# qianyizh/ElasticReconstruction

Hardware: AMD Instinct MI355X
Metric: depth frames/sec into 512^3 TSDF (640x480) (higher is better)
Workload: dtype f32; 1 GPU; configs[1]; frames_per_gpu=91800, volume_units_touched=122, warp=True, inputs=hbm_resident, parallelism=single GPU

## Files before the change

### elasticreconstruction_amd/_ffi.py

```python
import ctypes as C
import os

_HERE = os.path.dirname(os.path.abspath(__file__))
LIB_PATH = os.environ.get("ER_HIP_LIB") or os.path.join(_HERE, "liber_hip.so")

SYMBOLS = [
    "er_last_error", "er_device_count", "er_abi_version", "er_request_hw_queues", "er_host_alloc", "er_host_free", "er_host_copy_h2d", "er_device_alloc", "er_device_free", "er_device_copy_d2h",
    "er_tsdf_create", "er_tsdf_destroy", "er_tsdf_set_stream", "er_tsdf_synchronize",
    "er_tsdf_wait_event", "er_tsdf_reset", "er_tsdf_status", "er_tsdf_set_unit_shard", "er_unit_owner",
    "er_tsdf_scale_depth", "er_tsdf_reproject", "er_tsdf_integrate", "er_tsdf_integrate_frames", "er_tsdf_prepass_trace", "er_tsdf_set_zbuf_epoch",
    "er_tsdf_unit_count", "er_tsdf_unit_keys", "er_tsdf_read_unit", "er_tsdf_sum_weight",
    "er_tsdf_extract_world", "er_tsdf_extract_surface", "er_tsdf_extract_oriented", "er_tsdf_extract_mesh", "er_mc_table", "er_tsdf_extract_mesh_indexed", "er_mesh_components", "er_tsdf_extract_mesh_cleaned", "er_mesh_simplify", "er_tsdf_extract_mesh_simplified", "er_tsdf_import_world", "er_raycast_params_default", "er_tsdf_raycast", "er_tsdf_raycast_batch", "er_tsdf_export_weighted", "er_tsdf_import_weighted",
    "er_tsdf_export_raw", "er_tsdf_import_raw",
    "er_tsdf_color_enable", "er_tsdf_read_unit_color", "er_tsdf_write_unit_color", "er_tsdf_color_frames", "er_tsdf_reproject_color", "er_tsdf_sample_colors",
    "er_tsdf_band_sizes", "er_tsdf_export_band", "er_tsdf_merge_band", "er_tsdf_import_band", "er_tsdf_drop_units",
    "er_tsdf_set_profiling", "er_tsdf_get_profile", "er_tsdf_set_timeline", "er_tsdf_get_timeline",
    "er_comm_unique_id", "er_comm_create", "er_comm_create_local", "er_comm_create_loopback", "er_comm_destroy", "er_comm_rank", "er_comm_world",
    "er_tsdf_allreduce", "er_comm_merge_stats", "er_comm_merge_stats_owner", "er_frame_block",
    "er_cloud_create", "er_cloud_create_batch", "er_cloud_create_from_tsdf", "er_cloud_destroy", "er_cloud_size",
    "er_icp_count_inliers", "er_icp_align", "er_icp_align_trace", "er_find_correspondence",
    "er_icp_count_inliers_batch", "er_icp_align_batch", "er_find_correspondence_batch", "er_icp_release_workspaces", "er_registration_batch", "er_ransac_fitness_batch", "er_ransac_inliers",
    "er_features_create", "er_features_destroy", "er_features_size", "er_feature_knn", "er_ransac_hypotheses", "er_ransac_params_default", "er_ransac_align", "er_ransac_align_batch",
    "er_odom_params_default", "er_odom_create", "er_odom_destroy", "er_odom_align_pairs", "er_odom_track", "er_frame_to_model_align", "er_frames_to_models_align", "er_odom_linearize", "er_odom_read_maps", "er_odom_tables",
    "er_cloud_read", "er_cloud_voxel_grid", "er_cloud_estimate_normals", "er_fpfh_estimate", "er_features_dim", "er_features_read",
    "er_frag_params_default", "er_frag_create", "er_frag_destroy", "er_frag_lane_bytes", "er_frag_build", "er_frag_count", "er_frag_read",
# ... 72 lines not shown
    L.er_tsdf_create.argtypes = [C.c_int, C.c_int, fp, C.c_int, C.c_int, C.POINTER(vp)]
    L.er_tsdf_destroy.argtypes = [vp]
    L.er_tsdf_set_stream.argtypes = [vp, vp]
    L.er_tsdf_synchronize.argtypes = [vp]
    L.er_tsdf_wait_event.argtypes = [vp, vp]
    L.er_tsdf_reset.argtypes = [vp]
    L.er_tsdf_status.argtypes = [vp, ip, C.POINTER(C.c_long)]
    L.er_tsdf_set_unit_shard.argtypes = [vp, C.c_int, C.c_int]
    L.er_unit_owner.argtypes = [C.c_int, C.c_int]
    L.er_tsdf_scale_depth.argtypes = [vp, vp, vp]
    L.er_tsdf_reproject.argtypes = [vp, vp, vp, C.c_int, C.c_float, vp, vp]
    L.er_tsdf_integrate.argtypes = [vp, vp, vp]
    L.er_tsdf_integrate_frames.argtypes = [vp, C.c_int, vp, C.c_int, vp, C.POINTER(ErWarp)]
    if hasattr(L, "er_tsdf_prepass_trace"):
        L.er_tsdf_prepass_trace.argtypes = [vp, C.c_int, vp, C.c_int, vp, C.POINTER(ErWarp), vp, ip, vp, vp, vp, vp, vp, C.c_int, ip]
    if hasattr(L, "er_tsdf_set_zbuf_epoch"):
        L.er_tsdf_set_zbuf_epoch.argtypes = [vp, C.c_int, C.c_uint]
    L.er_tsdf_unit_count.argtypes = [vp, ip]
    L.er_tsdf_unit_keys.argtypes = [vp, vp]
    L.er_tsdf_read_unit.argtypes = [vp, C.c_int, vp, vp]
    L.er_tsdf_sum_weight.argtypes = [vp, dp]
    L.er_tsdf_extract_world.argtypes = [vp, vp, C.c_long, C.POINTER(C.c_long)]
    L.er_tsdf_extract_surface.argtypes = [vp, vp, C.c_long, C.POINTER(C.c_long)]
    if hasattr(L, "er_tsdf_extract_oriented"):
        L.er_tsdf_extract_oriented.argtypes = [vp, vp, vp, C.c_long, C.POINTER(C.c_long)]
    L.er_tsdf_extract_mesh.argtypes = [vp, vp, C.c_long, C.POINTER(C.c_long)]
    L.er_mc_table.argtypes = [vp]
    if hasattr(L, "er_tsdf_extract_mesh_indexed"):
        L.er_tsdf_extract_mesh_indexed.argtypes = [vp, vp, vp, C.c_long, vp, C.c_long, C.POINTER(C.c_long), C.POINTER(C.c_long)]
        L.er_tsdf_import_world.argtypes = [vp, vp, C.c_long, ip]
# ... 188 lines not shown
```

### elasticreconstruction_amd/csrc/er_tsdf.h

```cpp
#pragma once

#include "er_common.h"
#include "er_compact.h"
#include "er_mem.h"
#include "er_tsdf_math.h"

#include "../../include/er_hip.h"

#include <algorithm>
#include <cstdlib>
#include <functional>
#include <utility>
#include <vector>

namespace er_tsdf_k {
using namespace er;

constexpr int kBlock = 256;
constexpr int kEmptyKey = -1;
constexpr uint32_t kZEmpty = 0xFFFFFFFFu;
constexpr uint32_t kZEpochMax = 0xFFFFu;

enum { C_NUNITS = 0, C_NBATCH = 1 , C_POOL_OVERFLOW = 2, C_TABLE_FULL = 3, C_OUT_OF_RANGE = 4,
       C_NBATCH1 = 6, C_NBATCH2 = 7, C_ZERO_WRITE = 8 ,
// ... 39 lines not shown
    const uint16_t* __restrict__ depth, uint32_t* __restrict__ zbuf, int n_frames, int cols, int rows,
    Camera cam, CameraInv cami, const float* __restrict__ lambda, const double* __restrict__ T12, float* __restrict__ scaled,
    int* __restrict__ ht_key, int* __restrict__ ht_slot, unsigned long long* __restrict__ ht_mask, int cap_mask,
    int hash_shift, int* __restrict__ batch, int* __restrict__ nbatch,
    int* __restrict__ counters, float* __restrict__ tile_max, float* __restrict__ tile_lo, float* __restrict__ tile_lo_fine, int2 shard,
    uint32_t* __restrict__ lastzero, uint32_t* __restrict__ zfix, const int* __restrict__ zero_flag, uint32_t ztag);
extern template __global__ void k_prepare<true>(const uint16_t* __restrict__, uint32_t* __restrict__, int, int, int, Camera, CameraInv, const float* __restrict__, const double* __restrict__, float* __restrict__, int* __restrict__, int* __restrict__, unsigned long long* __restrict__, int, int, int* __restrict__, int* __restrict__, int* __restrict__, float* __restrict__, float* __restrict__, float* __restrict__, int2, uint32_t* __restrict__, uint32_t* __restrict__, const int* __restrict__, uint32_t);
extern template __global__ void k_prepare<false>(const uint16_t* __restrict__, uint32_t* __restrict__, int, int, int, Camera, CameraInv, const float* __restrict__, const double* __restrict__, float* __restrict__, int* __restrict__, int* __restrict__, unsigned long long* __restrict__, int, int, int* __restrict__, int* __restrict__, int* __restrict__, float* __restrict__, float* __restrict__, float* __restrict__, int2, uint32_t* __restrict__, uint32_t* __restrict__, const int* __restrict__, uint32_t);

constexpr int kRows = 4;
constexpr int kItemsPerUnit = 256;

struct Plan {
  int n_units;
  int next;
};

struct PlanRec {
  int key;
  int slot;
  unsigned long long mask;
};

constexpr int kIntMinBlocks = 5;

template <bool kSure>
__global__ __launch_bounds__(kBlock, kIntMinBlocks) void k_integrate(
    float2* __restrict__ pool, const PlanRec* __restrict__ plan_rec, Plan* __restrict__ plan,
    const FrameXform* __restrict__ frames, const float* __restrict__ scaled, const float* __restrict__ tile_max,
    const float* __restrict__ tile_lo, const float* __restrict__ tile_lo_fine, int tiles_x, int tiles_y, Camera cam, int cols, int rows);
extern template __global__ void k_integrate<true>(float2* __restrict__, const PlanRec* __restrict__, Plan* __restrict__, const FrameXform* __restrict__, const float* __restrict__, const float* __restrict__, const float* __restrict__, const float* __restrict__, int, int, Camera, int, int);
extern template __global__ void k_integrate<false>(float2* __restrict__, const PlanRec* __restrict__, Plan* __restrict__, const FrameXform* __restrict__, const float* __restrict__, const float* __restrict__, const float* __restrict__, const float* __restrict__, int, int, Camera, int, int);
}

struct er_tsdf_mem {
  er::DevScope fixed;
  er::Buffer<unsigned long long> color;
  er::Buffer<int> key_scratch, slot_scratch;
  er::Buffer<float> ctr_dev[2];
  er::Buffer<char> band_scratch;
  er::Buffer<char> color_scratch;
};

struct er_tsdf_s : er_tsdf_mem {
  int device = 0, cols = 0, rows = 0, pixels = 0, max_units = 0;
  er::Camera cam{};
  er::CameraInv cami{};
// ... 21 lines not shown
  er::PinnedBuffer<char> pinned[er_tsdf_k::kDepth];
  int ht_cap = 0, ht_shift = 0;
  float *lambda = nullptr, *ctr = nullptr;
  er::PinnedBuffer<float> ctr_pinned[2];
  hipEvent_t ctr_ev[2] = {nullptr, nullptr};
  hipEvent_t ctr_rd[2][er_tsdf_k::kAux] = {};
  bool ctr_rd_set[2] = {false, false};
  int ctr_parity = 0, ctr_cur = 0;
  uint16_t* depth_stage[er_tsdf_k::kDepth] = {};
  uint32_t *zbuf[er_tsdf_k::kAux] = {}, *lastzero[er_tsdf_k::kAux] = {}, *zfix[er_tsdf_k::kAux] = {};
  uint32_t zepoch[er_tsdf_k::kAux + 1] = {};
  double *T12 = nullptr, *seg12 = nullptr, *madj12 = nullptr, *dsum = nullptr;
  int* grid_index = nullptr;
  er_tsdf_k::PlanRec* plan_rec[er_tsdf_k::kDepth] = {};
  er_tsdf_k::Plan* plan[er_tsdf_k::kDepth] = {};
  int prof_stride = 0;
  long prof_tick = 0;
  std::vector<std::pair<hipEvent_t, hipEvent_t>> events;
  double ms_total = 0.0;
  long launches = 0, frames_done = 0;
  struct TimelineRow {
    long batch;
    int slot, stream, frames;
    double host_ms[3];
    hipEvent_t ev[7];
  };
  bool tl_on = false;
  hipEvent_t tl_base = nullptr;
  double tl_host0 = 0.0;
  std::vector<TimelineRow> tl_rows;
// ... 23 lines not shown
```

### elasticreconstruction_amd/csrc/er_tsdf.hip

```cpp
#include "er_tsdf_dev.h"

#include <chrono>
#include <climits>

namespace {

using namespace er_tsdf_k;

constexpr int kNbatchSlot[3] = {C_NBATCH, C_NBATCH1, C_NBATCH2};
constexpr int kZeroFlagSlot[2] = {C_ZERO_WRITE, C_ZERO_WRITE1};

__global__ void k_lambda(float* __restrict__ lambda, int cols, int rows, Camera cam) {
  int p = blockIdx.x * blockDim.x + threadIdx.x;
  if (p >= cols * rows) return;
  lambda[p] = scale_lambda(p % cols, p / cols, cam);
}

__global__ void k_scale_depth(const uint16_t* __restrict__ depth, const float* __restrict__ lambda,
                              float* __restrict__ scaled, int pixels, float itrunc) {
  int p = blockIdx.x * blockDim.x + threadIdx.x;
  if (p >= pixels) return;
  scaled[p] = scale_depth_px(depth[p], lambda[p], itrunc);
}

// ... 49 lines not shown
                                              int* __restrict__ zero_flag, unsigned long long* __restrict__ stats) {
  __shared__ int hist[65];
  __shared__ int start[66];
  const int n = *nbatch;
  for (int t = threadIdx.x; t < 65; t += blockDim.x) hist[t] = 0;
  __syncthreads();
  for (int t = threadIdx.x; t < n; t += blockDim.x) atomicAdd(&hist[__popcll(ht_mask[batch[t]])], 1);
  __syncthreads();
  if (threadIdx.x == 0) {
    int acc = 0;
    for (int c = 64; c >= 0; c--) {
      start[c] = acc;
      acc += hist[c];
    }
    plan->n_units = n;
    plan->next = 0;
    if (zero_flag) zero_flag[0] = zero_flag[1] = 0;
  }
  __syncthreads();
  if (threadIdx.x == 0) *nbatch = 0;
  unsigned long long visits = 0;
  for (int t = threadIdx.x; t < n; t += blockDim.x) {
    const int e = batch[t];
    const unsigned long long mask = ht_mask[e];
    ht_mask[e] = 0ull;
    visits += (unsigned long long)__popcll(mask);
    const int key = ht_key[e];
    PlanRec r;
    r.key = key;
    r.slot = unit_slot_acquire(e, key, ht_slot, unit_key, max_units, counters);
    r.mask = mask;
    plan_rec[atomicAdd(&start[__popcll(mask)], 1)] = r;
  }
  if (visits) atomicAdd(&stats[0], visits);
}

__global__ void k_sum_weight(const float2* __restrict__ pool, long n_vox, double* __restrict__ out) {
  double s = 0.0;
  for (long t = (long)blockIdx.x * blockDim.x + threadIdx.x; t < n_vox; t += (long)gridDim.x * blockDim.x)
    s += (double)pool[t].y;
  for (int off = 32; off > 0; off >>= 1) s += __shfl_down(s, off);
  __shared__ double part[kBlock / 64];
  if ((threadIdx.x & 63) == 0) part[threadIdx.x >> 6] = s;
  __syncthreads();
  if (threadIdx.x == 0) {
    double b = 0.0;
    for (int w = 0; w < kBlock / 64; w++) b += part[w];
    atomicAdd(out, b);
  }
// ... 218 lines not shown
      st->fx[f].mi[q] = (float)Tinv[q];
      st->t12[f * 12 + q] = Tf[q];
    }
    st->fx[f].tx = (float)Tf[3];
    st->fx[f].ty = (float)Tf[7];
    st->fx[f].tz = (float)Tf[11];
    st->fx[f].pad = 0.f;
    for (int q = 0; q < 16; q++) st->fxT[q][f] = reinterpret_cast<const float*>(&st->fx[f])[q];
  }
  static_assert(offsetof(Staging, fxT) == sizeof(er::FrameXform) * ER_MAX_BATCH && sizeof(er::FrameXform) == 64, "fxT lies directly behind fx");
  hipStream_t X = h->aux_stream[a], S = h->own_stream;
  int* nbatch = h->counters + kNbatchSlot[p];

  constexpr int kIntBlocksPerCu = 3;
  const int wide_grid = h->n_cu * kIntBlocksPerCu;
  uint32_t* zsrc = nullptr;
  char* dst = static_cast<char*>(h->dstage[p]);
  const double* dev_t12 = reinterpret_cast<const double*>(dst + offsetof(Staging, t12));
  const double* dev_seg = reinterpret_cast<const double*>(dst + offsetof(Staging, seg));
  const double* dev_madj = reinterpret_cast<const double*>(dst + offsetof(Staging, madj));
  const int* dev_gi = reinterpret_cast<const int*>(dst + offsetof(Staging, gi));
  if (warp) {
    for (int f = 0; f < n; f++) {
      for (int q = 0; q < 12; q++) {
        st->seg[f * 16 + q] = warp->seg[(size_t)(frame0 + f) * 16 + q];
        st->madj[f * 12 + q] = warp->madj[(size_t)(frame0 + f) * 16 + q];
      }
      er::cube_coord_deltas(&st->seg[f * 16], h->cam, h->cols, h->rows, &st->seg[f * 16 + 12]);
      st->seg[f * 16 + 15] = 0.0;
      const int g = warp->grid_index[frame0 + f];
// ... 18 lines not shown
    zsrc = h->zbuf[a];
  }
  if (tl && tl_record(h, &tl->ev[2], X)) return 1;

  const bool wide = h->cols % 4 == 0 && (zsrc || reinterpret_cast<uintptr_t>(depth_dev) % 8 == 0);
  hipLaunchKernelGGL(wide ? k_prepare<true> : k_prepare<false>, dim3((h->cols + kTile - 1) / kTile, (h->rows + kTile - 1) / kTile, n), dim3(kPrepThreads), 0, X,
                     depth_dev, zsrc, n, h->cols, h->rows, h->cam, h->cami, h->lambda, dev_t12, h->scaled[p], h->ht_key, h->ht_slot,
                     h->ht_mask[p], h->ht_cap - 1, h->ht_shift, h->batch[p], nbatch, h->counters,
                     h->tile_max[p], h->tile_lo[p], h->tile_lo_fine[p], make_int2(h->shard_rank, h->shard_world), h->lastzero[a], h->zfix[a],
                     h->counters + kZeroFlagSlot[a], ztag);
  if (tl && tl_record(h, &tl->ev[3], X)) return 1;
  hipLaunchKernelGGL(k_plan, dim3(1), dim3(256), 0, X, h->batch[p], nbatch, h->ht_mask[p], h->ht_key, h->ht_slot, h->unit_key, h->max_units,
                     h->counters, h->plan_rec[p], h->plan[p], warp ? h->counters + kZeroFlagSlot[a] : (int*)nullptr, h->stats);
  ER_HIP_TRY(hipGetLastError());
  if (tl && tl_record(h, &tl->ev[4], X)) return 1;
  ER_HIP_TRY(hipEventRecord(h->pre_done[p], X));

  ER_HIP_TRY(hipStreamWaitEvent(S, h->pre_done[p], 0));
  if (tl && tl_record(h, &tl->ev[5], S)) return 1;
  hipEvent_t e0 = nullptr, e1 = nullptr;
  const bool timed = h->prof_stride > 0 && (h->prof_tick++ % h->prof_stride) == 0;
  if (timed) {
    ER_HIP_TRY(hipEventCreate(&e0));
    ER_HIP_TRY(hipEventCreate(&e1));
    ER_HIP_TRY(hipEventRecord(e0, S));
  }
  const bool sure = h->cam.integration_trunc < 64.0f;
  hipLaunchKernelGGL(sure ? k_integrate<true> : k_integrate<false>, dim3(wide_grid), dim3(kBlock), 0, S, h->pool, h->plan_rec[p], h->plan[p],
                     h->frames[p], h->scaled[p], h->tile_max[p], h->tile_lo[p], h->tile_lo_fine[p], (h->cols + kTile - 1) / kTile, (h->rows + kTile - 1) / kTile,
                     h->cam, h->cols, h->rows);
  if (timed) {
    ER_HIP_TRY(hipEventRecord(e1, S));
    h->events.emplace_back(e0, e1);
  }
  ER_HIP_TRY(hipGetLastError());
  if (tl && tl_record(h, &tl->ev[6], S)) return 1;
  ER_HIP_TRY(hipEventRecord(h->int_done[p], S));
  h->used[p] = true;
  h->frames_done += n;
  if (tl) tl->host_ms[2] = host_now_ms() - h->tl_host0;
  return 0;
}

}

// ... 75 lines not shown
  for (int q = 0; q < kDepth; q++) bad = bad || M.alloc(&h->depth_stage[q], B * px, who);
  for (int q = 0; q < kAux; q++) bad = bad || M.alloc(&h->zbuf[q], B * px, who);
  for (int q = 0; q < kAux; q++) bad = bad || M.alloc(&h->lastzero[q], B * px, who);
  for (int q = 0; q < kAux; q++) bad = bad || M.alloc(&h->zfix[q], B * px, who);
  for (int q = 0; q < kDepth; q++) bad = bad || M.alloc(&h->dstage[q], sizeof(Staging), who);
  bad = bad || M.alloc(&h->T12, B * 12, who);
  bad = bad || M.alloc(&h->seg12, B * 16, who);
  bad = bad || M.alloc(&h->madj12, B * 12, who);
  bad = bad || M.alloc(&h->grid_index, B, who);
  bad = bad || M.alloc(&h->dsum, 1, who);
  for (int q = 0; q < kDepth; q++) bad = bad || M.alloc(&h->tile_max[q], tiles, who);
  for (int q = 0; q < kDepth; q++) bad = bad || M.alloc(&h->tile_lo[q], tiles, who);
  for (int q = 0; q < kDepth; q++) bad = bad || M.alloc(&h->tile_lo_fine[q], tiles_fine, who);
  for (int q = 0; q < kDepth; q++) bad = bad || M.alloc(&h->plan_rec[q], (size_t)cap, who);
  for (int q = 0; q < kDepth; q++) bad = bad || M.alloc(&h->plan[q], 1, who);
  if (bad) {
    er_tsdf_destroy(h);
    return 1;
  }
  for (int q = 0; q < kDepth; q++) h->frames[q] = reinterpret_cast<er::FrameXform*>(reinterpret_cast<char*>(h->dstage[q]) + offsetof(Staging, fx));
  hipStream_t s = h->stream;
  bool ok = hipMemsetAsync(h->pool, 0, (size_t)max_units * er::kUnitVox * sizeof(float2), s) == hipSuccess &&
            hipMemsetAsync(h->ht_key, 0xFF, (size_t)cap * sizeof(int), s) == hipSuccess &&
            hipMemsetAsync(h->ht_slot, 0xFF, (size_t)cap * sizeof(int), s) == hipSuccess &&
            hipMemsetAsync(h->counters, 0, C_COUNT * sizeof(int), s) == hipSuccess &&
            hipMemsetAsync(h->stats, 0, 4 * sizeof(unsigned long long), s) == hipSuccess;
  for (int q = 0; q < kDepth; q++)
    ok = ok && hipMemsetAsync(h->ht_mask[q], 0, (size_t)cap * sizeof(unsigned long long), s) == hipSuccess &&
         hipMemsetAsync(h->scaled[q], 0, B * (px + kScaledPad) * sizeof(float), s) == hipSuccess;
  for (int q = 0; q < kAux; q++)
// ... 229 lines not shown
  ER_HIP_TRY(hipMemcpy(&plan, h->plan[p], sizeof plan, hipMemcpyDeviceToHost));
  if (plan.n_units < 0 || plan.n_units > h->ht_cap) return er::fail("er_tsdf_prepass_trace: the batch lists %d units", plan.n_units);
  if (n_keys) *n_keys = plan.n_units;
  if (keys || masks) {
    std::vector<PlanRec> rec((size_t)plan.n_units);
    if (plan.n_units > 0) ER_HIP_TRY(hipMemcpy(rec.data(), h->plan_rec[p], rec.size() * sizeof(PlanRec), hipMemcpyDeviceToHost));
    std::sort(rec.begin(), rec.end(), [](const PlanRec& a, const PlanRec& b) { return a.key < b.key; });
    for (int i = 0; i < plan.n_units && i < keys_cap; i++) {
      if (keys) keys[i] = rec[(size_t)i].key;
      if (masks) masks[i] = rec[(size_t)i].mask;
    }
  }
  return 0;
}

int er_tsdf_set_zbuf_epoch(er_tsdf_t h, int which, unsigned epoch) {
  if (!h) return er::fail("er_tsdf_set_zbuf_epoch: NULL handle");
  if (which < 0 || which > kZColor) return er::fail("er_tsdf_set_zbuf_epoch: no z-buffer %d (0, 1: the pre-pass streams'; %d: the colour calls')", which, kZColor);
  if (epoch > kZEpochMax) return er::fail("er_tsdf_set_zbuf_epoch: epoch %u above %u", epoch, kZEpochMax);
  ER_HIP_TRY(hipSetDevice(h->device));
  if (sync_all(h)) return 1;
  if (which < kAux && epoch < h->zepoch[which]) {
    ER_HIP_TRY(hipMemsetAsync(h->zbuf[which], 0xFF, (size_t)ER_MAX_BATCH * (size_t)h->pixels * sizeof(uint32_t), h->stream));
    ER_HIP_TRY(hipStreamSynchronize(h->stream));
  }
  h->zepoch[which] = epoch;
  return 0;
}

int er_tsdf_wait_event(er_tsdf_t h, void* hip_event) {
// ... 201 lines not shown
```

### elasticreconstruction_amd/csrc/er_tsdf_int.hip

```cpp
#include "er_tsdf.h"

namespace er_tsdf_k {

template <bool kSure>
__global__ __launch_bounds__(kBlock, kIntMinBlocks) void k_integrate(
    float2* __restrict__ pool, const PlanRec* __restrict__ plan_rec, Plan* __restrict__ plan,
    const FrameXform* __restrict__ frames, const float* __restrict__ scaled, const float* __restrict__ tile_max,
    const float* __restrict__ tile_lo, const float* __restrict__ tile_lo_fine, int tiles_x, int tiles_y, Camera cam, int cols, int rows) {
  const int lane = threadIdx.x & 63;
  const int wave = threadIdx.x >> 6;
  const int pixels = cols * rows;
  const int lo_tiles_x = (cols + (1 << kLoShift) - 1) >> kLoShift;
  const int n_items = plan->n_units * kItemsPerUnit;
  __shared__ int s_item;
  for (;;) {
    __syncthreads();
    if (threadIdx.x == 0) s_item = atomicAdd(&plan->next, 1);
    __syncthreads();
    const int item = s_item;
    if (item >= n_items) break;
    const PlanRec rec = plan_rec[item >> 8];
    const int ilane = lane >> 5;
    const int i = ((item >> 5) & 7) * 8 + ilane;
    const int j0 = ((item >> 2) & 7) * 8 + (wave >> 1) * 4;
    const int jlane = (lane >> 3) & 3, k0 = (item & 3) * 16 + (wave & 1) * 8, klane = lane & 7;
    constexpr int jspan = 4, kspan = 8, ispan = 2 * kRows, istep = 2;
    const int ibox = i - ilane;
    const int key = rec.key, slot = rec.slot;
    if (slot < 0) continue;
    unsigned long long m = rec.mask;
    const int xi = key >> 18, yi = (key >> 9) & 511, zi = key & 511;
    const float xs = unit_shift(xi), ys = unit_shift(yi), zs = unit_shift(zi);
    const float g2 = grid_coord(k0 + klane, zs);
    float2* __restrict__ slab = pool + (size_t)slot * kUnitVox + (size_t)i * (kUnitRes * kUnitRes) + (j0 + jlane) * kUnitRes + k0 + klane;
    float S[kRows], W[kRows], W0[kRows], g0[kRows];
    const float g1 = grid_coord(j0 + jlane, ys);
#pragma unroll
    for (int r = 0; r < kRows; r++) g0[r] = grid_coord(i + r * istep, xs);
    constexpr int row_stride = istep * kUnitRes * kUnitRes;
#pragma unroll
    for (int r = 0; r < kRows; r++) {
      const float2 v = slab[r * row_stride];
      S[r] = v.x;
      W[r] = v.y;
      W0[r] = v.y;
    }
    unsigned long long m_in, m_full;
    {
      bool keep = ((m >> lane) & 1ull) != 0ull, inside = false, full = false;
      FrameXform fl;
      if (keep) {
        const float* __restrict__ fT = reinterpret_cast<const float*>(frames + ER_MAX_BATCH) + lane;
#pragma unroll
        for (int q = 0; q < 12; q++) fl.mi[q] = fT[q * ER_MAX_BATCH];
        fl.tx = fT[12 * ER_MAX_BATCH];
        fl.ty = fT[13 * ER_MAX_BATCH];
        fl.tz = fT[14 * ER_MAX_BATCH];
        fl.pad = 0.f;
      }
      if (keep)
        keep = patch_may_update_box(grid_coord(ibox, xs), grid_coord(ibox + ispan - 1, xs), grid_coord(j0, ys), grid_coord(j0 + jspan - 1, ys),
                                    grid_coord(k0, zs), grid_coord(k0 + kspan - 1, zs), fl, cam, cols, rows,
                                    tile_max + lane, tiles_x, tiles_y, &inside, tile_lo + lane, &full, kLoShift, lo_tiles_x, tile_lo_fine + lane,
                                    ER_MAX_BATCH);
      m = __ballot(keep);
      m_in = __ballot(keep && inside);
      m_full = __ballot(keep && full);
    }
    auto project = [&](int f, float (&dp)[kRows]) {
      const FrameXform fx = frames[f];
      const float* __restrict__ sc = scaled + (size_t)f * (pixels + kScaledPad);
      unsigned pix[kRows];
      if ((m_in >> f) & 1ull) {
#pragma unroll
        for (int r = 0; r < kRows; r++) pix[r] = voxel_project_inside(g0[r], g1, g2, fx, cam, cols, rows);
      } else
      {
#pragma unroll
        for (int r = 0; r < kRows; r++) {
          unsigned pixel;
          const bool ok = voxel_project(g0[r], g1, g2, fx, cam, cols, rows, pixel);
          pix[r] = ok ? pixel : (unsigned)pixels;
// ... 84 lines not shown
          project(nf, dpa);
          finish(pf, dpb);
          pf = nf;
        }
        float dpl[kRows];
#pragma unroll
        for (int r = 0; r < kRows; r++) dpl[r] = last_in_b ? dpb[r] : dpa[r];
        finish(pf, dpl);
      }
      runs_before(64);
    }
#pragma unroll
    for (int r = 0; r < kRows; r++)
      if (W[r] != W0[r]) slab[r * row_stride] = make_float2(S[r], W[r]);
  }
}
template __global__ void k_integrate<true>(float2* __restrict__, const PlanRec* __restrict__, Plan* __restrict__, const FrameXform* __restrict__, const float* __restrict__, const float* __restrict__, const float* __restrict__, const float* __restrict__, int, int, Camera, int, int);
template __global__ void k_integrate<false>(float2* __restrict__, const PlanRec* __restrict__, Plan* __restrict__, const FrameXform* __restrict__, const float* __restrict__, const float* __restrict__, const float* __restrict__, const float* __restrict__, int, int, Camera, int, int);

}
```

### elasticreconstruction_amd/tsdf.py

```python
import ctypes as C
import os

import numpy as np

from . import _ffi
from . import formats

UNIT_VOX = 64 * 64 * 64


def mat4_mul(A, B):
    A = np.asarray(A, np.float64)
    B = np.asarray(B, np.float64)
    out = np.empty((4, 4), np.float64)
    for r in range(4):
        for c in range(4):
            out[r, c] = ((A[r, 0] * B[0, c] + A[r, 1] * B[1, c]) + A[r, 2] * B[2, c]) + A[r, 3] * B[3, c]
    return out


class TSDFVolume:

    def __init__(self, cols=640, rows=480, camera=None, max_units=1024, device=0):
        self._lib = _ffi.lib()
# ... 107 lines not shown
        fx, fy = (self.cols_ + 15) // 16, (self.rows_ + 15) // 16
        pad, nk = C.c_int(0), C.c_int(0)
        pad_floats = 64
        scaled = np.empty((n, px + pad_floats), np.float32)
        tmax, tlo = np.empty((ty, tx, B), np.float32), np.empty((ty, tx, B), np.float32)
        fine = np.empty((fy, fx, B), np.float32)
        cap = 1 << 16
        keys, masks = np.empty(cap, np.int32), np.empty(cap, np.uint64)
        _ffi.check(self._lib.er_tsdf_prepass_trace(self._h, n, src, on_dev, _ffi.ptr(T), w_ref, _ffi.ptr(scaled), C.byref(pad), _ffi.ptr(tmax),
                                                   _ffi.ptr(tlo), _ffi.ptr(fine), _ffi.ptr(keys), _ffi.ptr(masks), cap, C.byref(nk)),
                   "er_tsdf_prepass_trace")
        del keep
        assert pad.value == pad_floats and nk.value <= cap
        return dict(scaled=scaled, pad=pad.value, tile_max=tmax[:, :, :n].copy(), tile_lo=tlo[:, :, :n].copy(),
                    tile_lo_fine=fine[:, :, :n].copy(), keys=keys[:nk.value].copy(), masks=masks[:nk.value].copy())

    def set_zbuf_epoch(self, which, epoch):
        _ffi.check(self._lib.er_tsdf_set_zbuf_epoch(self._h, int(which), int(epoch)), "er_tsdf_set_zbuf_epoch")

    def unit_count(self):
        n = C.c_int(0)
        _ffi.check(self._lib.er_tsdf_unit_count(self._h, C.byref(n)), "er_tsdf_unit_count")
        return n.value

    def unit_keys(self):
        n = self.unit_count()
        keys = np.empty(n, dtype=np.int32)
        if n:
            _ffi.check(self._lib.er_tsdf_unit_keys(self._h, _ffi.ptr(keys)), "er_tsdf_unit_keys")
        return keys
# ... 451 lines not shown
```

### include/er_hip.h

```cpp
#ifndef ER_HIP_H_
#define ER_HIP_H_

#include <stddef.h>
#include <stdint.h>

#ifdef __cplusplus
extern "C" {
#endif

#define ER_UNIT_RES 64
#define ER_UNIT_VOX (64 * 64 * 64)
#define ER_MAX_BATCH 64

const char* er_last_error(void);
int er_device_count(void);
int er_abi_version(void);
int er_request_hw_queues(int n);

void* er_host_alloc(size_t bytes);
int er_host_free(void* p);
int er_host_copy_h2d(void* dev_dst, const void* host_src, size_t bytes);
void* er_device_alloc(size_t bytes, int device);
int er_device_free(void* p);
int er_device_copy_d2h(void* host_dst, const void* dev_src, size_t bytes);
// ... 17 lines not shown
int er_tsdf_synchronize(er_tsdf_t h);

int er_tsdf_scale_depth(er_tsdf_t h, const uint16_t* depth_host, float* scaled_host);

int er_tsdf_reproject(er_tsdf_t h, uint16_t* depth_inout_host, const float* ctr_host, int resolution, float length,
                      const double seg[16], const double madj[16]);

int er_tsdf_integrate(er_tsdf_t h, const uint16_t* depth_host, const double T[16]);

int er_tsdf_integrate_frames(er_tsdf_t h, int n, const uint16_t* depth, int depth_on_device, const double* T,
                             const er_warp* warp);

int er_tsdf_prepass_trace(er_tsdf_t h, int n, const uint16_t* depth, int depth_on_device, const double* T, const er_warp* warp,
                          float* scaled, int* scaled_pad, float* tile_max, float* tile_lo, float* tile_lo_fine,
                          int* keys, unsigned long long* masks, int keys_cap, int* n_keys);

int er_tsdf_set_zbuf_epoch(er_tsdf_t h, int which, unsigned epoch);

int er_tsdf_wait_event(er_tsdf_t h, void* hip_event);

int er_tsdf_reset(er_tsdf_t h);

#define ER_STATUS_POOL_EXHAUSTED 1
#define ER_STATUS_TABLE_FULL 2
int er_tsdf_status(er_tsdf_t h, int* flags, long* out_of_range_pixels);

int er_tsdf_unit_count(er_tsdf_t h, int* count);
int er_tsdf_unit_keys(er_tsdf_t h, int* keys_host);
int er_tsdf_read_unit(er_tsdf_t h, int key, float* sdf_host, float* weight_host);

// ... 298 lines not shown
```

Baseline: 200,800 frames/s.

## Precompute per-item box verdicts and cost-sort the integration work queue

Splits the frustum/box culling out of the integrate kernel into a new verdict kernel that stores per-wave masks and a per-item cost. A single-block ordering kernel then builds a queue sorted by descending cost and skips zero-cost items, so the integrate kernel pulls expensive items first and never visits empty ones. The aim is better load balance across the dynamic work queue and less per-item culling work in the hot kernel. In exchange it adds two extra launches on the pre-pass stream, a serial single-block sort over all units, and extra memory traffic for box records. A trace API and optional per-workgroup timing instrumentation are also added.

After: 198,300 frames/s. -1.2%, worse.

```diff
diff --git a/elasticreconstruction_amd/_ffi.py b/elasticreconstruction_amd/_ffi.py
--- a/elasticreconstruction_amd/_ffi.py
+++ b/elasticreconstruction_amd/_ffi.py
@@ -8,7 +8,7 @@
     "er_last_error", "er_device_count", "er_abi_version", "er_request_hw_queues", "er_host_alloc", "er_host_free", "er_host_copy_h2d", "er_device_alloc", "er_device_free", "er_device_copy_d2h",
     "er_tsdf_create", "er_tsdf_destroy", "er_tsdf_set_stream", "er_tsdf_synchronize",
     "er_tsdf_wait_event", "er_tsdf_reset", "er_tsdf_status", "er_tsdf_set_unit_shard", "er_unit_owner",
-    "er_tsdf_scale_depth", "er_tsdf_reproject", "er_tsdf_integrate", "er_tsdf_integrate_frames", "er_tsdf_prepass_trace", "er_tsdf_set_zbuf_epoch",
+    "er_tsdf_scale_depth", "er_tsdf_reproject", "er_tsdf_integrate", "er_tsdf_integrate_frames", "er_tsdf_prepass_trace", "er_tsdf_queue_trace", "er_tsdf_set_zbuf_epoch",
     "er_tsdf_unit_count", "er_tsdf_unit_keys", "er_tsdf_read_unit", "er_tsdf_sum_weight",
     "er_tsdf_extract_world", "er_tsdf_extract_surface", "er_tsdf_extract_oriented", "er_tsdf_extract_mesh", "er_mc_table", "er_tsdf_extract_mesh_indexed", "er_mesh_components", "er_tsdf_extract_mesh_cleaned", "er_mesh_simplify", "er_tsdf_extract_mesh_simplified", "er_tsdf_import_world", "er_raycast_params_default", "er_tsdf_raycast", "er_tsdf_raycast_batch", "er_tsdf_export_weighted", "er_tsdf_import_weighted",
     "er_tsdf_export_raw", "er_tsdf_import_raw",
@@ -111,6 +111,8 @@
     L.er_tsdf_integrate_frames.argtypes = [vp, C.c_int, vp, C.c_int, vp, C.POINTER(ErWarp)]
     if hasattr(L, "er_tsdf_prepass_trace"):
         L.er_tsdf_prepass_trace.argtypes = [vp, C.c_int, vp, C.c_int, vp, C.POINTER(ErWarp), vp, ip, vp, vp, vp, vp, vp, C.c_int, ip]
+    if hasattr(L, "er_tsdf_queue_trace"):
+        L.er_tsdf_queue_trace.argtypes = [vp, C.c_int, vp, C.c_int, vp, C.POINTER(ErWarp), vp, vp, vp, vp, vp, C.c_int, ip, vp, C.c_int, ip]
     if hasattr(L, "er_tsdf_set_zbuf_epoch"):
         L.er_tsdf_set_zbuf_epoch.argtypes = [vp, C.c_int, C.c_uint]
     L.er_tsdf_unit_count.argtypes = [vp, ip]
diff --git a/elasticreconstruction_amd/csrc/er_queue_order.h b/elasticreconstruction_amd/csrc/er_queue_order.h
--- /dev/null
+++ b/elasticreconstruction_amd/csrc/er_queue_order.h
@@ -0,0 +1,28 @@
+#pragma once
+
+#include "er_tsdf_math.h"
+
+namespace er {
+
+constexpr int kQueueCosts = 65;
+
+ER_HD int box_cost(unsigned long long m, unsigned long long m_full) {
+  const int c = __builtin_popcountll(m & ~m_full);
+  return c > 0 ? c : (m != 0ull ? 1 : 0);
+}
+
+ER_HD int queue_starts(const int* hist, int* start) {
+  int acc = 0;
+  for (int c = kQueueCosts - 1; c >= 1; c--) {
+    start[c] = acc;
+    acc += hist[c];
+  }
+  start[0] = acc;
+  return acc;
+}
+
+ER_HD unsigned queue_entry(int unit_rank, int item) { return ((unsigned)unit_rank << 8) | (unsigned)item; }
+ER_HD int entry_unit(unsigned e) { return (int)(e >> 8); }
+ER_HD int entry_item(unsigned e) { return (int)(e & 255u); }
+
+}
diff --git a/elasticreconstruction_amd/csrc/er_tsdf.h b/elasticreconstruction_amd/csrc/er_tsdf.h
--- a/elasticreconstruction_amd/csrc/er_tsdf.h
+++ b/elasticreconstruction_amd/csrc/er_tsdf.h
@@ -3,6 +3,7 @@
 #include "er_common.h"
 #include "er_compact.h"
 #include "er_mem.h"
+#include "er_queue_order.h"
 #include "er_tsdf_math.h"
 
 #include "../../include/er_hip.h"
@@ -77,6 +78,7 @@
 struct Plan {
   int n_units;
   int next;
+  int n_items;
 };
 
 struct PlanRec {
@@ -85,15 +87,23 @@
   unsigned long long mask;
 };
 
+struct BoxRec {
+  unsigned long long m, m_in, m_full, pad;
+};
+
 constexpr int kIntMinBlocks = 5;
+
+__global__ __launch_bounds__(kBlock) void k_verdict(
+    const PlanRec* __restrict__ plan_rec, const Plan* __restrict__ plan, const FrameXform* __restrict__ frames, const float* __restrict__ tile_max,
+    const float* __restrict__ tile_lo, const float* __restrict__ tile_lo_fine, int tiles_x, int tiles_y, Camera cam, int cols, int rows,
+    BoxRec* __restrict__ box_rec, unsigned char* __restrict__ item_cost);
 
 template <bool kSure>
 __global__ __launch_bounds__(kBlock, kIntMinBlocks) void k_integrate(
-    float2* __restrict__ pool, const PlanRec* __restrict__ plan_rec, Plan* __restrict__ plan,
-    const FrameXform* __restrict__ frames, const float* __restrict__ scaled, const float* __restrict__ tile_max,
-    const float* __restrict__ tile_lo, const float* __restrict__ tile_lo_fine, int tiles_x, int tiles_y, Camera cam, int cols, int rows);
-extern template __global__ void k_integrate<true>(float2* __restrict__, const PlanRec* __restrict__, Plan* __restrict__, const FrameXform* __restrict__, const float* __restrict__, const float* __restrict__, const float* __restrict__, const float* __restrict__, int, int, Camera, int, int);
-extern template __global__ void k_integrate<false>(float2* __restrict__, const PlanRec* __restrict__, Plan* __restrict__, const FrameXform* __restrict__, const float* __restrict__, const float* __restrict__, const float* __restrict__, const float* __restrict__, int, int, Camera, int, int);
+    float2* __restrict__ pool, const PlanRec* __restrict__ plan_rec, Plan* __restrict__ plan, const BoxRec* __restrict__ box_rec,
+    const unsigned* __restrict__ item_order, const FrameXform* __restrict__ frames, const float* __restrict__ scaled, Camera cam, int cols, int rows);
+extern template __global__ void k_integrate<true>(float2* __restrict__, const PlanRec* __restrict__, Plan* __restrict__, const BoxRec* __restrict__, const unsigned* __restrict__, const FrameXform* __restrict__, const float* __restrict__, Camera, int, int);
+extern template __global__ void k_integrate<false>(float2* __restrict__, const PlanRec* __restrict__, Plan* __restrict__, const BoxRec* __restrict__, const unsigned* __restrict__, const FrameXform* __restrict__, const float* __restrict__, Camera, int, int);
 }
 
 struct er_tsdf_mem {
@@ -145,6 +155,9 @@
   int* grid_index = nullptr;
   er_tsdf_k::PlanRec* plan_rec[er_tsdf_k::kDepth] = {};
   er_tsdf_k::Plan* plan[er_tsdf_k::kDepth] = {};
+  er_tsdf_k::BoxRec* box_rec[er_tsdf_k::kDepth] = {};
+  unsigned char* item_cost[er_tsdf_k::kDepth] = {};
+  unsigned* item_order[er_tsdf_k::kDepth] = {};
   int prof_stride = 0;
   long prof_tick = 0;
   std::vector<std::pair<hipEvent_t, hipEvent_t>> events;
diff --git a/elasticreconstruction_amd/csrc/er_tsdf.hip b/elasticreconstruction_amd/csrc/er_tsdf.hip
--- a/elasticreconstruction_amd/csrc/er_tsdf.hip
+++ b/elasticreconstruction_amd/csrc/er_tsdf.hip
@@ -87,7 +87,6 @@
       acc += hist[c];
     }
     plan->n_units = n;
-    plan->next = 0;
     if (zero_flag) zero_flag[0] = zero_flag[1] = 0;
   }
   __syncthreads();
@@ -106,6 +105,34 @@
     plan_rec[atomicAdd(&start[__popcll(mask)], 1)] = r;
   }
   if (visits) atomicAdd(&stats[0], visits);
+}
+
+__global__ __launch_bounds__(kItemsPerUnit) void k_order(const PlanRec* __restrict__ plan_rec, Plan* __restrict__ plan,
+                                                         const unsigned char* __restrict__ item_cost, unsigned* __restrict__ item_order) {
+  __shared__ int hist[kQueueCosts];
+  __shared__ int start[kQueueCosts];
+  const int n_units = plan->n_units;
+  auto cost_of = [&](int u) {
+    const int slot = plan_rec[u].slot;
+    const int c = slot >= 0 ? (int)item_cost[(size_t)slot * kItemsPerUnit + threadIdx.x] : 0;
+    return c < kQueueCosts ? c : kQueueCosts - 1;
+  };
+  for (int t = threadIdx.x; t < kQueueCosts; t += blockDim.x) hist[t] = 0;
+  __syncthreads();
+  for (int u = 0; u < n_units; u++) {
+    const int c = cost_of(u);
+    if (c) atomicAdd(&hist[c], 1);
+  }
+  __syncthreads();
+  if (threadIdx.x == 0) {
+    plan->n_items = queue_starts(hist, start);
+    plan->next = 0;
+  }
+  __syncthreads();
+  for (int u = 0; u < n_units; u++) {
+    const int c = cost_of(u);
+    if (c) item_order[atomicAdd(&start[c], 1)] = queue_entry(u, (int)threadIdx.x);
+  }
 }
 
 __global__ void k_sum_weight(const float2* __restrict__ pool, long n_vox, double* __restrict__ out) {
@@ -354,6 +381,7 @@
 
   constexpr int kIntBlocksPerCu = 3;
   const int wide_grid = h->n_cu * kIntBlocksPerCu;
+  constexpr int kVerdictBlocksPerCu = 4;
   uint32_t* zsrc = nullptr;
   char* dst = static_cast<char*>(h->dstage[p]);
   const double* dev_t12 = reinterpret_cast<const double*>(dst + offsetof(Staging, t12));
@@ -402,6 +430,11 @@
                      h->counters, h->plan_rec[p], h->plan[p], warp ? h->counters + kZeroFlagSlot[a] : (int*)nullptr, h->stats);
   ER_HIP_TRY(hipGetLastError());
   if (tl && tl_record(h, &tl->ev[4], X)) return 1;
+  const int tiles_x = (h->cols + kTile - 1) / kTile, tiles_y = (h->rows + kTile - 1) / kTile;
+  hipLaunchKernelGGL(k_verdict, dim3(h->n_cu * kVerdictBlocksPerCu), dim3(kBlock), 0, X, h->plan_rec[p], h->plan[p], h->frames[p], h->tile_max[p],
+                     h->tile_lo[p], h->tile_lo_fine[p], tiles_x, tiles_y, h->cam, h->cols, h->rows, h->box_rec[p], h->item_cost[p]);
+  hipLaunchKernelGGL(k_order, dim3(1), dim3(kItemsPerUnit), 0, X, h->plan_rec[p], h->plan[p], h->item_cost[p], h->item_order[p]);
+  ER_HIP_TRY(hipGetLastError());
   ER_HIP_TRY(hipEventRecord(h->pre_done[p], X));
 
   ER_HIP_TRY(hipStreamWaitEvent(S, h->pre_done[p], 0));
@@ -415,8 +448,7 @@
   }
   const bool sure = h->cam.integration_trunc < 64.0f;
   hipLaunchKernelGGL(sure ? k_integrate<true> : k_integrate<false>, dim3(wide_grid), dim3(kBlock), 0, S, h->pool, h->plan_rec[p], h->plan[p],
-                     h->frames[p], h->scaled[p], h->tile_max[p], h->tile_lo[p], h->tile_lo_fine[p], (h->cols + kTile - 1) / kTile, (h->rows + kTile - 1) / kTile,
-                     h->cam, h->cols, h->rows);
+                     h->box_rec[p], h->item_order[p], h->frames[p], h->scaled[p], h->cam, h->cols, h->rows);
   if (timed) {
     ER_HIP_TRY(hipEventRecord(e1, S));
     h->events.emplace_back(e0, e1);
@@ -522,6 +554,9 @@
   for (int q = 0; q < kDepth; q++) bad = bad || M.alloc(&h->tile_lo_fine[q], tiles_fine, who);
   for (int q = 0; q < kDepth; q++) bad = bad || M.alloc(&h->plan_rec[q], (size_t)cap, who);
   for (int q = 0; q < kDepth; q++) bad = bad || M.alloc(&h->plan[q], 1, who);
+  for (int q = 0; q < kDepth; q++) bad = bad || M.alloc(&h->box_rec[q], (size_t)max_units * kItemsPerUnit * (kBlock / 64), who);
+  for (int q = 0; q < kDepth; q++) bad = bad || M.alloc(&h->item_cost[q], (size_t)max_units * kItemsPerUnit, who);
+  for (int q = 0; q < kDepth; q++) bad = bad || M.alloc(&h->item_order[q], (size_t)max_units * kItemsPerUnit, who);
   if (bad) {
     er_tsdf_destroy(h);
     return 1;
@@ -781,6 +816,52 @@
   return 0;
 }
 
+int er_tsdf_queue_trace(er_tsdf_t h, int n, const uint16_t* depth, int depth_on_device, const double* T, const er_warp* warp,
+                        int* keys, int* slots, unsigned long long* masks, unsigned long long* box, unsigned char* cost, int units_cap,
+                        int* n_units, unsigned* queue, int queue_cap, int* n_queue) {
+  if (!h || !n_units || !n_queue) return er::fail("er_tsdf_queue_trace: NULL argument");
+  if (n < 1 || n > ER_MAX_BATCH) return er::fail("er_tsdf_queue_trace: %d frames outside 1..%d (one batch)", n, ER_MAX_BATCH);
+  ER_HIP_TRY(hipSetDevice(h->device));
+  if (sync_all(h)) return 1;
+  const int p = (int)(h->batch_no % kDepth);
+  if (er_tsdf_integrate_frames(h, n, depth, depth_on_device, T, warp)) return 1;
+  if (sync_all(h)) return 1;
+  Plan plan{};
+  ER_HIP_TRY(hipMemcpy(&plan, h->plan[p], sizeof plan, hipMemcpyDeviceToHost));
+  if (plan.n_units < 0 || plan.n_units > h->ht_cap || plan.n_items < 0 || (size_t)plan.n_items > (size_t)h->max_units * kItemsPerUnit)
+    return er::fail("er_tsdf_queue_trace: the batch lists %d units and %d items", plan.n_units, plan.n_items);
+  *n_units = plan.n_units;
+  *n_queue = plan.n_items;
+  std::vector<PlanRec> rec((size_t)plan.n_units);
+  if (plan.n_units > 0) ER_HIP_TRY(hipMemcpy(rec.data(), h->plan_rec[p], rec.size() * sizeof(PlanRec), hipMemcpyDeviceToHost));
+  constexpr int kWaves = kBlock / 64;
+  std::vector<BoxRec> br((size_t)kItemsPerUnit * kWaves);
+  for (int u = 0; u < plan.n_units && u < units_cap; u++) {
+    const PlanRec& r = rec[(size_t)u];
+    if (keys) keys[u] = r.key;
+    if (slots) slots[u] = r.slot;
+    if (masks) masks[u] = r.mask;
+    const bool held = r.slot >= 0 && r.slot < h->max_units;
+    if (box) {
+      unsigned long long* b = box + (size_t)u * kItemsPerUnit * kWaves * 3;
+      if (held) ER_HIP_TRY(hipMemcpy(br.data(), h->box_rec[p] + (size_t)r.slot * br.size(), br.size() * sizeof(BoxRec), hipMemcpyDeviceToHost));
+      for (size_t i = 0; i < br.size(); i++) {
+        b[3 * i] = held ? br[i].m : 0ull;
+        b[3 * i + 1] = held ? br[i].m_in : 0ull;
+        b[3 * i + 2] = held ? br[i].m_full : 0ull;
+      }
+    }
+    if (cost) {
+      unsigned char* c = cost + (size_t)u * kItemsPerUnit;
+      if (held) ER_HIP_TRY(hipMemcpy(c, h->item_cost[p] + (size_t)r.slot * kItemsPerUnit, kItemsPerUnit, hipMemcpyDeviceToHost));
+      else memset(c, 0, kItemsPerUnit);
+    }
+  }
+  const int nq = std::min(plan.n_items, queue_cap);
+  if (queue && nq > 0) ER_HIP_TRY(hipMemcpy(queue, h->item_order[p], (size_t)nq * sizeof(unsigned), hipMemcpyDeviceToHost));
+  return 0;
+}
+
 int er_tsdf_set_zbuf_epoch(er_tsdf_t h, int which, unsigned epoch) {
   if (!h) return er::fail("er_tsdf_set_zbuf_epoch: NULL handle");
   if (which < 0 || which > kZColor) return er::fail("er_tsdf_set_zbuf_epoch: no z-buffer %d (0, 1: the pre-pass streams'; %d: the colour calls')", which, kZColor);
diff --git a/elasticreconstruction_amd/csrc/er_tsdf_int.hip b/elasticreconstruction_amd/csrc/er_tsdf_int.hip
--- a/elasticreconstruction_amd/csrc/er_tsdf_int.hip
+++ b/elasticreconstruction_amd/csrc/er_tsdf_int.hip
@@ -2,49 +2,27 @@
 
 namespace er_tsdf_k {
 
-template <bool kSure>
-__global__ __launch_bounds__(kBlock, kIntMinBlocks) void k_integrate(
-    float2* __restrict__ pool, const PlanRec* __restrict__ plan_rec, Plan* __restrict__ plan,
-    const FrameXform* __restrict__ frames, const float* __restrict__ scaled, const float* __restrict__ tile_max,
-    const float* __restrict__ tile_lo, const float* __restrict__ tile_lo_fine, int tiles_x, int tiles_y, Camera cam, int cols, int rows) {
+__global__ __launch_bounds__(kBlock) void k_verdict(
+    const PlanRec* __restrict__ plan_rec, const Plan* __restrict__ plan, const FrameXform* __restrict__ frames, const float* __restrict__ tile_max,
+    const float* __restrict__ tile_lo, const float* __restrict__ tile_lo_fine, int tiles_x, int tiles_y, Camera cam, int cols, int rows,
+    BoxRec* __restrict__ box_rec, unsigned char* __restrict__ item_cost) {
   const int lane = threadIdx.x & 63;
   const int wave = threadIdx.x >> 6;
-  const int pixels = cols * rows;
   const int lo_tiles_x = (cols + (1 << kLoShift) - 1) >> kLoShift;
   const int n_items = plan->n_units * kItemsPerUnit;
-  __shared__ int s_item;
-  for (;;) {
-    __syncthreads();
-    if (threadIdx.x == 0) s_item = atomicAdd(&plan->next, 1);
-    __syncthreads();
-    const int item = s_item;
-    if (item >= n_items) break;
-    const PlanRec rec = plan_rec[item >> 8];
-    const int ilane = lane >> 5;
-    const int i = ((item >> 5) & 7) * 8 + ilane;
-    const int j0 = ((item >> 2) & 7) * 8 + (wave >> 1) * 4;
-    const int jlane = (lane >> 3) & 3, k0 = (item & 3) * 16 + (wave & 1) * 8, klane = lane & 7;
-    constexpr int jspan = 4, kspan = 8, ispan = 2 * kRows, istep = 2;
-    const int ibox = i - ilane;
+  __shared__ int s_cost[kBlock / 64];
+  for (int it = blockIdx.x; it < n_items; it += gridDim.x) {
+    const PlanRec rec = plan_rec[it >> 8];
+    const int item = it & (kItemsPerUnit - 1);
     const int key = rec.key, slot = rec.slot;
     if (slot < 0) continue;
     unsigned long long m = rec.mask;
     const int xi = key >> 18, yi = (key >> 9) & 511, zi = key & 511;
     const float xs = unit_shift(xi), ys = unit_shift(yi), zs = unit_shift(zi);
-    const float g2 = grid_coord(k0 + klane, zs);
-    float2* __restrict__ slab = pool + (size_t)slot * kUnitVox + (size_t)i * (kUnitRes * kUnitRes) + (j0 + jlane) * kUnitRes + k0 + klane;
-    float S[kRows], W[kRows], W0[kRows], g0[kRows];
-    const float g1 = grid_coord(j0 + jlane, ys);
-#pragma unroll
-    for (int r = 0; r < kRows; r++) g0[r] = grid_coord(i + r * istep, xs);
-    constexpr int row_stride = istep * kUnitRes * kUnitRes;
-#pragma unroll
-    for (int r = 0; r < kRows; r++) {
-      const float2 v = slab[r * row_stride];
-      S[r] = v.x;
-      W[r] = v.y;
-      W0[r] = v.y;
-    }
+    const int j0 = ((item >> 2) & 7) * 8 + (wave >> 1) * 4;
+    const int k0 = (item & 3) * 16 + (wave & 1) * 8;
+    constexpr int jspan = 4, kspan = 8, ispan = 2 * kRows;
+    const int ibox = ((item >> 5) & 7) * 8;
     unsigned long long m_in, m_full;
     {
       bool keep = ((m >> lane) & 1ull) != 0ull, inside = false, full = false;
@@ -66,6 +44,83 @@
       m = __ballot(keep);
       m_in = __ballot(keep && inside);
       m_full = __ballot(keep && full);
+    }
+    const size_t at = (size_t)slot * kItemsPerUnit + (size_t)item;
+    if (lane == 0) {
+      box_rec[at * (kBlock / 64) + wave] = BoxRec{m, m_in, m_full, 0ull};
+      s_cost[wave] = box_cost(m, m_full);
+    }
+    __syncthreads();
+    if (threadIdx.x == 0) {
+      int c = s_cost[0];
+#pragma unroll
+      for (int w = 1; w < kBlock / 64; w++) c = s_cost[w] > c ? s_cost[w] : c;
+      item_cost[at] = (unsigned char)c;
+    }
+    __syncthreads();
+  }
+}
+
+#ifdef ER_WG_TRACE
+constexpr int kWgTraceLaunches = 64, kWgTraceMaxWg = 2048;
+__device__ unsigned long long er_wg_trace_buf[kWgTraceLaunches][kWgTraceMaxWg][4];
+__device__ unsigned er_wg_trace_exits;
+#endif
+
+template <bool kSure>
+__global__ __launch_bounds__(kBlock, kIntMinBlocks) void k_integrate(
+    float2* __restrict__ pool, const PlanRec* __restrict__ plan_rec, Plan* __restrict__ plan, const BoxRec* __restrict__ box_rec,
+    const unsigned* __restrict__ item_order, const FrameXform* __restrict__ frames, const float* __restrict__ scaled, Camera cam, int cols, int rows) {
+  const int lane = threadIdx.x & 63;
+  const int wave = threadIdx.x >> 6;
+  const int pixels = cols * rows;
+  const int n_items = plan->n_items;
+  __shared__ int s_item;
+#ifdef ER_WG_TRACE
+  const unsigned long long wt_start = wall_clock64();
+  unsigned long long wt_claimed = wt_start, wt_longest = 0ull, wt_items = 0ull;
+#endif
+  for (;;) {
+    __syncthreads();
+    if (threadIdx.x == 0) s_item = atomicAdd(&plan->next, 1);
+    __syncthreads();
+    const int pos = s_item;
+#ifdef ER_WG_TRACE
+    {
+      const unsigned long long now = wall_clock64();
+      if (wt_items && now - wt_claimed > wt_longest) wt_longest = now - wt_claimed;
+      wt_claimed = now;
+      if (pos < n_items) wt_items++;
+    }
+#endif
+    if (pos >= n_items) break;
+    const unsigned entry = item_order[pos];
+    const int item = entry_item(entry);
+    const PlanRec rec = plan_rec[entry_unit(entry)];
+    const int ilane = lane >> 5;
+    const int i = ((item >> 5) & 7) * 8 + ilane;
+    const int j0 = ((item >> 2) & 7) * 8 + (wave >> 1) * 4;
+    const int jlane = (lane >> 3) & 3, k0 = (item & 3) * 16 + (wave & 1) * 8, klane = lane & 7;
+    constexpr int istep = 2;
+    const int key = rec.key, slot = rec.slot;
+    const BoxRec box = box_rec[((size_t)slot * kItemsPerUnit + (size_t)item) * (kBlock / 64) + (size_t)__builtin_amdgcn_readfirstlane(wave)];
+    const unsigned long long m = box.m, m_in = box.m_in, m_full = box.m_full;
+    if (m == 0ull) continue;
+    const int xi = key >> 18, yi = (key >> 9) & 511, zi = key & 511;
+    const float xs = unit_shift(xi), ys = unit_shift(yi), zs = unit_shift(zi);
+    const float g2 = grid_coord(k0 + klane, zs);
+    float2* __restrict__ slab = pool + (size_t)slot * kUnitVox + (size_t)i * (kUnitRes * kUnitRes) + (j0 + jlane) * kUnitRes + k0 + klane;
+    float S[kRows], W[kRows], W0[kRows], g0[kRows];
+    const float g1 = grid_coord(j0 + jlane, ys);
+#pragma unroll
+    for (int r = 0; r < kRows; r++) g0[r] = grid_coord(i + r * istep, xs);
+    constexpr int row_stride = istep * kUnitRes * kUnitRes;
+#pragma unroll
+    for (int r = 0; r < kRows; r++) {
+      const float2 v = slab[r * row_stride];
+      S[r] = v.x;
+      W[r] = v.y;
+      W0[r] = v.y;
     }
     auto project = [&](int f, float (&dp)[kRows]) {
       const FrameXform fx = frames[f];
@@ -180,8 +235,29 @@
     for (int r = 0; r < kRows; r++)
       if (W[r] != W0[r]) slab[r * row_stride] = make_float2(S[r], W[r]);
   }
-}
-template __global__ void k_integrate<true>(float2* __restrict__, const PlanRec* __restrict__, Plan* __restrict__, const FrameXform* __restrict__, const float* __restrict__, const float* __restrict__, const float* __restrict__, const float* __restrict__, int, int, Camera, int, int);
-template __global__ void k_integrate<false>(float2* __restrict__, const PlanRec* __restrict__, Plan* __restrict__, const FrameXform* __restrict__, const float* __restrict__, const float* __restrict__, const float* __restrict__, const float* __restrict__, int, int, Camera, int, int);
-
-}
+#ifdef ER_WG_TRACE
+  if (threadIdx.x == 0 && gridDim.x <= (unsigned)kWgTraceMaxWg) {
+    const unsigned e = atomicAdd(&er_wg_trace_exits, 1u);
+    unsigned long long* o = er_wg_trace_buf[(e / gridDim.x) % kWgTraceLaunches][e % gridDim.x];
+    o[0] = wt_start;
+    o[1] = wall_clock64();
+    o[2] = wt_items;
+    o[3] = wt_longest;
+  }
+#endif
+}
+template __global__ void k_integrate<true>(float2* __restrict__, const PlanRec* __restrict__, Plan* __restrict__, const BoxRec* __restrict__, const unsigned* __restrict__, const FrameXform* __restrict__, const float* __restrict__, Camera, int, int);
+template __global__ void k_integrate<false>(float2* __restrict__, const PlanRec* __restrict__, Plan* __restrict__, const BoxRec* __restrict__, const unsigned* __restrict__, const FrameXform* __restrict__, const float* __restrict__, Camera, int, int);
+
+}
+
+#ifdef ER_WG_TRACE
+extern "C" int er_wg_trace_read(unsigned long long* out, unsigned* exits, int reset) {
+  using namespace er_tsdf_k;
+  if (out) ER_HIP_TRY(hipMemcpyFromSymbol(out, HIP_SYMBOL(er_wg_trace_buf), sizeof(unsigned long long) * kWgTraceLaunches * kWgTraceMaxWg * 4));
+  if (exits) ER_HIP_TRY(hipMemcpyFromSymbol(exits, HIP_SYMBOL(er_wg_trace_exits), sizeof(unsigned)));
+  const unsigned zero = 0u;
+  if (reset) ER_HIP_TRY(hipMemcpyToSymbol(HIP_SYMBOL(er_wg_trace_exits), &zero, sizeof zero));
+  return 0;
+}
+#endif
diff --git a/elasticreconstruction_amd/tsdf.py b/elasticreconstruction_amd/tsdf.py
--- a/elasticreconstruction_amd/tsdf.py
+++ b/elasticreconstruction_amd/tsdf.py
@@ -145,6 +145,26 @@
         assert pad.value == pad_floats and nk.value <= cap
         return dict(scaled=scaled, pad=pad.value, tile_max=tmax[:, :, :n].copy(), tile_lo=tlo[:, :, :n].copy(),
                     tile_lo_fine=fine[:, :, :n].copy(), keys=keys[:nk.value].copy(), masks=masks[:nk.value].copy())
+
+    def queue_trace(self, depth, transformations, warp=None):
+        T = np.ascontiguousarray(transformations, dtype=np.float64).reshape(-1, 16)
+        n = T.shape[0]
+        w_ref, keep = self._warp_ref(warp, n)
+        d = np.ascontiguousarray(depth, dtype=np.uint16).reshape(n, -1)
+        assert d.shape[1] == self.cols_ * self.rows_
+        cap = 64
+        keys, slots, masks = np.empty(cap, np.int32), np.empty(cap, np.int32), np.empty(cap, np.uint64)
+        box, cost = np.empty((cap, 256, 4, 3), np.uint64), np.empty((cap, 256), np.uint8)
+        queue = np.empty(cap * 256, np.uint32)
+        nu, nq = C.c_int(0), C.c_int(0)
+        _ffi.check(self._lib.er_tsdf_queue_trace(self._h, n, _ffi.ptr(d), 0, _ffi.ptr(T), w_ref, _ffi.ptr(keys), _ffi.ptr(slots), _ffi.ptr(masks),
+                                                 _ffi.ptr(box), _ffi.ptr(cost), cap, C.byref(nu), _ffi.ptr(queue), cap * 256, C.byref(nq)),
+                   "er_tsdf_queue_trace")
+        assert nu.value <= cap and nq.value <= cap * 256, "the batch touches %d units: more than this wrapper provides for" % nu.value
+        del keep
+        u, q = nu.value, nq.value
+        return dict(keys=keys[:u].copy(), slots=slots[:u].copy(), masks=masks[:u].copy(), box=box[:u].copy(), cost=cost[:u].copy(),
+                    queue=queue[:q].copy())
 
     def set_zbuf_epoch(self, which, epoch):
         _ffi.check(self._lib.er_tsdf_set_zbuf_epoch(self._h, int(which), int(epoch)), "er_tsdf_set_zbuf_epoch")
diff --git a/include/er_hip.h b/include/er_hip.h
--- a/include/er_hip.h
+++ b/include/er_hip.h
@@ -55,6 +55,10 @@
 int er_tsdf_prepass_trace(er_tsdf_t h, int n, const uint16_t* depth, int depth_on_device, const double* T, const er_warp* warp,
                           float* scaled, int* scaled_pad, float* tile_max, float* tile_lo, float* tile_lo_fine,
                           int* keys, unsigned long long* masks, int keys_cap, int* n_keys);
+
+int er_tsdf_queue_trace(er_tsdf_t h, int n, const uint16_t* depth, int depth_on_device, const double* T, const er_warp* warp,
+                        int* keys, int* slots, unsigned long long* masks, unsigned long long* box, unsigned char* cost, int units_cap,
+                        int* n_units, unsigned* queue, int queue_cap, int* n_queue);
 
 int er_tsdf_set_zbuf_epoch(er_tsdf_t h, int which, unsigned epoch);
 
```
